# mlvlab/BLiM

Measured on AMD Instinct MI355X. Metric: candidate-pairs/sec (7B, 96+32 tok), higher is better.
Workload: dtype f16; 1 GPU; SYN v2t-VTG re-rank: Qwen2-7B dims (28 layers), seeded synthetic weights, 96 video + 32 text tokens per pair, top-16 text candidates per video query, 55 queries (880 pairs, 32560 packed tokens, 28160 label rows) per step per GPU; prefix_reuse=True, vtg_compensated=none, parallelism=query rows sharded over 1 GPU(s); RCCL all-gather of score rows at the end

## Files before the change

blim_amd/csrc/engine.hip:

```cpp
#include <math.h>
#include <stdarg.h>
#include <stdio.h>
#include <stdlib.h>
#include <string.h>

#include <algorithm>
#include <map>
#include <string>
#include <vector>

#include "engine.hpp"

static thread_local char g_err[1024] = "";
void blim_set_error(const char* fmt, ...) {
    va_list ap;
    va_start(ap, fmt);
    vsnprintf(g_err, sizeof(g_err), fmt, ap);
    va_end(ap);
}
extern "C" const char* blim_last_error(void) { return g_err; }
extern "C" int blim_abi_version(void) { return BLIM_ABI_VERSION; }

static const char* kTimeClassNames[TC_COUNT] = {"gemm_qkv_rope", "attention", "gemm_o_resid", "gemm_gateup_swiglu", "gemm_down_resid",
                                                "rmsnorm", "lm_head_lse", "gemm_other", "misc", "quantize_fp8"};
// ... 1406 lines not shown
        hipEventDestroy(s.a); hipEventDestroy(s.b);
    }
    e->spans.clear();
    return BLIM_OK;
}
extern "C" int blim_debug_read(blim_engine* e, const char* which, void* dst, int64_t bytes, void* stream) {
    ARG_CHECK(e && which && dst && bytes > 0);
    const DevBuf* b = nullptr;
    if (!strcmp(which, "resid")) b = &e->resid;
    else if (!strcmp(which, "xn")) b = &e->xn;
    else if (!strcmp(which, "qkv")) b = &e->qkv;
    else if (!strcmp(which, "attn")) b = &e->attn;
    else if (!strcmp(which, "act")) b = &e->act;
    else if (!strcmp(which, "act8")) b = &e->act8;
    else if (!strcmp(which, "act_mx")) b = &e->act_mx;
    if (!b || !b->p || (size_t)bytes > b->bytes) { blim_set_error("debug_read: no buffer '%s' of %lld bytes", which, (long long)bytes); return BLIM_ERR_ARG; }
    HIP_TRY(hipMemcpyAsync(dst, b->p, (size_t)bytes, hipMemcpyDeviceToDevice, (hipStream_t)stream));
    return BLIM_OK;
}
extern "C" int blim_debug_gemm_stamps(void* device_buf) {
    gemm_set_debug_stamps((unsigned long long*)device_buf);
    return BLIM_OK;
}
extern "C" int blim_set_option(blim_engine* e, const char* key, int32_t value) {
    ARG_CHECK(e && key);
    if (!strcmp(key, "attn_tr_read")) { e->attn_tr = value; return BLIM_OK; }
    if (!strcmp(key, "f8_mask")) { e->f8_mask = value & 31; return BLIM_OK; }
    if (!strcmp(key, "f8_fuse")) { e->f8_fuse = value != 0; return BLIM_OK; }
    if (!strcmp(key, "precise_embeds")) { e->precise_embeds = value != 0; return BLIM_OK; }
    if (!strcmp(key, "prune_last")) { e->prune_last = value != 0; return BLIM_OK; }
    if (!strcmp(key, "masked_query_zero")) {
        if (value && e->f8) { blim_set_error("option 'masked_query_zero' needs a 16-bit engine (the fp8 mode's attention output leaves the kernel quantised)"); return BLIM_ERR_ARG; }
        e->masked_query_zero = value != 0; return BLIM_OK;
    }
    if (!strcmp(key, "precise_lo6")) {
        if (value && e->f8) { blim_set_error("option 'precise_lo6' needs a 16-bit engine (fp16: the default; bf16: opt-in)"); return BLIM_ERR_ARG; }
        if (value && (e->c.hidden_size % 128 || e->c.intermediate_size % 128 || e->c.hidden_size > 20480 || e->c.intermediate_size > 20480)) {
            blim_set_error("option 'precise_lo6': hidden and intermediate sizes must be multiples of 128, at most 20480"); return BLIM_ERR_ARG; }
        if (value && e->aug && e->aug % 128) { blim_set_error("option 'precise_lo6': adapters were loaded with a %d-column K extension; set the option before loading adapters", e->aug); return BLIM_ERR_STATE; }
        e->lo6 = value != 0; return BLIM_OK;
    }
    if (!strcmp(key, "precise_mlp")) { e->precise_mlp = value != 0; return BLIM_OK; }
    if (!strcmp(key, "precise_layers")) {
        if (value && e->f8) { blim_set_error("option 'precise_layers' needs a 16-bit engine (fp16 or bf16)"); return BLIM_ERR_ARG; }
        e->layer_mask_on = value != 0; return BLIM_OK;
    }
// ... 16 lines not shown
```

blim_amd/csrc/gemm.hip:

```cpp
#include "gemm.hpp"
#include "kernels.hpp"
#include <type_traits>

#define BM 256
#define BN 256
#define BK 64
#define NTHREADS 512
#define TILE_BYTES (BM * BK * 2)
#define BUF_BYTES (2 * TILE_BYTES)
#define GROUP_M 8

typedef const __attribute__((address_space(1))) void* gptr_t;
typedef __attribute__((address_space(3))) void* lptr_t;

__device__ __forceinline__ void glds16(const void* g, char* lds_wave_base) {
    __builtin_amdgcn_global_load_lds((gptr_t)g, (lptr_t)lds_wave_base, 16, 0, 0);
}

__device__ __forceinline__ float gelu_erf(float x) {
    const float z = fabsf(x) * 0.70710678118654752f;
    const float t = __builtin_amdgcn_rcpf(fmaf(0.3275911f, z, 1.0f));
    const float poly = t * fmaf(t, fmaf(t, fmaf(t, fmaf(t, 1.061405429f, -1.453152027f), 1.421413741f), -0.284496736f), 0.254829592f);
    const float erf_abs = 1.0f - poly * __expf(-z * z);
    return 0.5f * x * (1.0f + copysignf(erf_abs, x));
}
__device__ __forceinline__ float silu_f(float x) { return x * __builtin_amdgcn_rcpf(1.0f + __expf(-x)); }

template <int EPI, int DT, bool SPLIT = false, bool MXA = false>
__global__ __launch_bounds__(NTHREADS) void gemm_kernel(const GemmParams p) {
    __shared__ __attribute__((aligned(16))) char smem[5 * TILE_BYTES];

    constexpr bool LO6_BF16_FENCE = MXA && DT == DT_BF16;
    const int tid = threadIdx.x;
    const int lane = tid & 63;
    const int wave = __builtin_amdgcn_readfirstlane(tid >> 6);
    const int wm = wave >> 2, wn = wave & 3;
    int stamp_vb = blockIdx.x;
    auto stamp = [&](int k) __attribute__((always_inline)) {
        if (p.debug_stamps && tid == 0) p.debug_stamps[(size_t)stamp_vb * 8 + k] = __builtin_amdgcn_s_memrealtime();
    };
    const int ntm = (p.M + BM - 1) / BM, ntn = (p.N + BN - 1) / BN;
    const int nwg = ntm * ntn;
#pragma unroll 1
    for (int vb = blockIdx.x; vb < (p.tile_map ? ((nwg + 255) & ~255) : nwg); vb += gridDim.x) {
    int pid;
    if (p.tile_map) {
        const int xcd = vb & 7, k = vb >> 3;
        pid = ((k >> 5) * 8 + xcd) * 32 + (k & 31);
        if (pid >= nwg) continue;
    } else {
        const int bid = vb, xcd = bid & 7, q = nwg >> 3, r = nwg & 7;
        pid = (xcd < r ? xcd * (q + 1) : r * (q + 1) + (xcd - r) * q) + (bid >> 3);
    }
    stamp_vb = pid;
    stamp(0);
    if constexpr (out16<DT>::value == DT_F16 || (LO6_BF16_FENCE)) { if (p.f16_saturate) f16_saturate_off(); }
    const int width = p.group_m * ntn;
    const int first_m = (pid / width) * p.group_m;
    const int gsz = min(ntm - first_m, p.group_m);
    const int tm = first_m + (pid % width) % gsz;
    const int tn = (pid % width) / gsz;
    const int row0 = tm * BM, col0 = tn * BN;

    const int sr = lane >> 3;
    const char* baseA = (const char*)p.A;
    const char* baseW = (const char*)p.W;

    constexpr int ES = (DT == DT_F8) ? 1 : 2;
    constexpr bool MX8 = MXA && DT == DT_F8;
    constexpr bool LO6 = MXA && DT != DT_F8;
    constexpr int ODT = out16<DT>::value;
    const int fr = lane & 15, fc = lane >> 4;
    const int fg = (fr >> 1) & 7;
    const int frag_off = (fr >> 3) * 1024 + (fr & 7) * 128 + 16 * ((fc ^ (fg & 3)) + 4 * (fg >> 2));
    const int a_off = (16 * wm) * 1024 + frag_off;
    const int b_off = (8 * wn) * 1024 + frag_off;

    f32x4 acc[8][4];
#pragma unroll
    for (int i = 0; i < 8; ++i)
#pragma unroll
        for (int j = 0; j < 4; ++j) acc[i][j] = (f32x4){0.f, 0.f, 0.f, 0.f};

    const int nk = p.K * ES / (BK * 2);
    const int nk6 = LO6 ? p.K6 / 128 : 0;
    float f8_scale = 0.f;
    if constexpr (DT == DT_F8) f8_scale = tid < 256 ? (p.row_scale ? p.row_scale[min(row0 + tid, p.M - 1)] : 1.0f) : p.col_scale[min(col0 + tid - 256, p.N - 1)];
    stamp(1);
    {
        const int grp = wave >> 2;
        typedef int i32x8 __attribute__((ext_vector_type(8)));
        typedef int i32x4 __attribute__((ext_vector_type(4)));
        bf16x8 fa[2][8], fb[2][4];
        i32x8 fa8[8], fb8[4];
        auto load_frags = [&](int offA_tile, int offB_tile) __attribute__((always_inline)) {
            const char* ba[2] = {smem + (offA_tile + a_off), smem + ((offA_tile + a_off) ^ 64)};
            const char* bb[2] = {smem + (offB_tile + b_off), smem + ((offB_tile + b_off) ^ 64)};
            if constexpr (DT == DT_F8) {
                auto rd = [](const char* q0, const char* q1) __attribute__((always_inline)) {
                    const i32x4 l = *(const i32x4*)q0, h = *(const i32x4*)q1;
                    return (i32x8){l[0], l[1], l[2], l[3], h[0], h[1], h[2], h[3]};
                };
#pragma unroll
                for (int ni = 0; ni < 4; ++ni) fb8[ni] = rd(bb[0] + ni * 2048, bb[1] + ni * 2048);
#pragma unroll
                for (int mi = 0; mi < 8; ++mi) fa8[mi] = rd(ba[0] + mi * 2048, ba[1] + mi * 2048);
            } else {
#pragma unroll
// ... 54 lines not shown
        const int sc = (lane & 7) ^ (4 * (wg & 1) + (sr >> 1));
        uint32_t off8[8];
#pragma unroll
        for (int i = 0; i < 8; ++i) {
            const int b = wg + 4 * i;
            if (grp == 1) off8[i] = (uint32_t)((int64_t)min(row0 + 8 * b + sr, p.M - 1) * p.lda * ES + 16 * sc);
            else off8[i] = (uint32_t)((int64_t)min(col0 + 8 * b + sr, p.N - 1) * (p.w_wrap_k > 0 ? p.w_wrap_k : p.K) * ES + 16 * sc);
        }
        const char* gbase = grp == 1 ? baseA : baseW;
        const int wrap = (grp == 0 && p.w_wrap_k > 0) ? p.w_wrap_k * ES / (BK * 2) : 0x7fffffff;
        auto stage8 = [&](int dst, int kt) __attribute__((always_inline)) {
#ifdef GEMM_ABLATE_DMA
            if (GEMM_ABLATE_DMA == 1 && kt >= 2) return;
            if (GEMM_ABLATE_DMA == 2) kt &= 1;
#endif
            const char* g = gbase + (int64_t)(kt >= wrap ? kt - wrap : kt) * (BK * 2);
#pragma unroll
            for (int i = 0; i < 8; ++i) {
                uint32_t o = off8[i];
                asm volatile("" : "+v"(o));
                glds16(g + o, smem + dst + (wg + 4 * i) * 1024);
            }
        };
        auto frags_and_dma = [&](int offA_tile, int offB_tile, int dst, int kt, bool on) __attribute__((always_inline)) {
            const char* ba[2] = {smem + (offA_tile + a_off), smem + ((offA_tile + a_off) ^ 64)};
            const char* bb[2] = {smem + (offB_tile + b_off), smem + ((offB_tile + b_off) ^ 64)};
#ifdef GEMM_ABLATE_DMA
            if (GEMM_ABLATE_DMA == 1 && kt >= 2) on = false;
            if (GEMM_ABLATE_DMA == 2) kt &= 1;
#endif
#if defined(GEMM_ABLATE_WREAD) && GEMM_ABLATE_WREAD == 2
            if (grp == 0 && kt >= 4) on = false;
#endif
            const char* g = gbase + (int64_t)(kt >= wrap ? kt - wrap : kt) * (BK * 2);
            auto dma1 = [&](int q) __attribute__((always_inline)) {
                __builtin_amdgcn_sched_barrier(0);
                if (on) { uint32_t o = off8[q]; asm volatile("" : "+v"(o)); glds16(g + o, smem + dst + (wg + 4 * q) * 1024); }
                __builtin_amdgcn_sched_barrier(0);
            };
            {
#pragma unroll
                for (int q = 0; q < 8; ++q) {
#pragma unroll
                    for (int j = 3 * q; j < 3 * q + 3; ++j) {
                        const int ks = j / 12, r = j % 12;
#ifdef GEMM_ABLATE_WREAD
                        if (r < 4) { }
#else
                        if (r < 4) fb[ks][r] = *(const bf16x8*)(bb[ks] + r * 2048);
#endif
                        else fa[ks][r - 4] = *(const bf16x8*)(ba[ks] + (r - 4) * 2048);
                    }
                    dma1(q);
                }
#ifdef GEMM_ABLATE_WREAD
#pragma unroll
                for (int ks = 0; ks < 2; ++ks)
#pragma unroll
                    for (int r = 0; r < 4; ++r) fb[ks][r] = fa[ks][r + 4];
#endif
            }
        };
        typedef int i32x2 __attribute__((ext_vector_type(2)));
        const char* g6A = LO6 ? (const char*)p.A6 + (int64_t)tm * nk6 * F6_TILE_BYTES : nullptr;
        const char* g6W = LO6 ? (const char*)p.W6 + (int64_t)tn * nk6 * F6_TILE_BYTES : nullptr;
        uint2 sc6a = make_uint2(0, 0);
        uint32_t sc6w = 0;
        auto dma6 = [&](int q, int dslot, int kd, bool isW, bool on) __attribute__((always_inline)) {
#if defined(GEMM_ABLATE_P2) && GEMM_ABLATE_P2 == 3
            on = on && kd < 3;
#endif
#if defined(GEMM_ABLATE_P2) && GEMM_ABLATE_P2 >= 4
            on = on && !((q == 4 || q == 5) && (isW || GEMM_ABLATE_P2 == 5));
#endif
            if (on) {
                const char* g = (isW ? g6W : g6A) + (int64_t)kd * F6_TILE_BYTES;
                char* d = smem + dslot * F6_TILE_BYTES;
                uint32_t o16 = (uint32_t)lane * 16u;
                asm volatile("" : "+v"(o16));
                if (q < 6) glds16(g + (wg + 4 * q) * 1024 + o16, d + (wg + 4 * q) * 1024);
                else if (lane < 16) glds16(g + 24576 + wg * 256 + o16, d + 24576 + wg * 256);
            }
        };
// ... 35 lines not shown
            stage8(TILE_BYTES, 0);
            if (nk > 1) stage8(3 * TILE_BYTES, 1);
            if (nk > 1) asm volatile("s_waitcnt vmcnt(8)" ::: "memory");
            else asm volatile("s_waitcnt vmcnt(0)" ::: "memory");
            PHASE_BARRIER();
            if constexpr (MX8) mx_cur = mx_nxt;
            if constexpr (DT == DT_F8) {
                int sp = 0;
                for (int k = 0; k < nk; ++k) {
                    mx_request(k + 1);
                    load_frags(sa, adv(sa, 1));
                    if (k >= 1 && k + 1 < nk) stage8(sp, k + 1);
                    PHASE_BARRIER();
                    compute();
                    asm volatile("s_waitcnt vmcnt(0)" ::: "memory");
                    if constexpr (MX8) mx_cur = mx_nxt;
                    PHASE_BARRIER();
                    sp = sa; sa = adv(sa, 2);
                }
                PHASE_BARRIER();
            } else {
            load_frags(0, TILE_BYTES);
            PHASE_BARRIER();
            for (int kt = 0; kt < nk; ++kt) {
                WP_T(0);
                compute();
                WP_T(1);
                asm volatile("s_waitcnt vmcnt(0)" ::: "memory");
                WP_T(2);
                PHASE_BARRIER();
                WP_T(3);
                if constexpr (LO6) { if (kt + 1 == nk) break; }
                if (kt + 1 < nk) frags_and_dma(adv(sa, 2), adv(sa, 3), sa, kt + 2, kt + 2 < nk);
#ifdef GEMM_WAIT_PROF
                asm volatile("s_waitcnt lgkmcnt(0)" ::: "memory");
#endif
                WP_T(4);
                PHASE_BARRIER();
                WP_T(5);
                WP_ACC();
                sa = adv(sa, 2);
            }
            if constexpr (LO6) {
                stage6(0, 0, false); stage6(1, 0, true);
                if (nk6 > 1) { stage6(2, 1, false); stage6(3, 1, true); }
                if (nk6 > 2) { stage6(4, 2, false); stage6(5, 2, true); }
                PHASE_BARRIER();
            }
            }
        } else {
            stage8(0, 0);
            if (nk > 1) stage8(2 * TILE_BYTES, 1);
            if (nk > 1) asm volatile("s_waitcnt vmcnt(8)" ::: "memory");
            else asm volatile("s_waitcnt vmcnt(0)" ::: "memory");
            PHASE_BARRIER();
            if constexpr (MX8) mx_cur = mx_nxt;
            PHASE_BARRIER();
            for (int kt = 0; kt < nk; ++kt) {
                WP_T(0);
                if constexpr (DT == DT_F8) {
                    mx_request(kt + 1);
                    load_frags(sa, adv(sa, 1));
                    if (kt + 2 < nk) stage8(adv(sa, 4), kt + 2);
                } else frags_and_dma(sa, adv(sa, 1), adv(sa, 4), kt + 2, kt + 2 < nk);
#ifdef GEMM_WAIT_PROF
                asm volatile("s_waitcnt lgkmcnt(0)" ::: "memory");
#endif
                WP_T(1);
                if (kt + 2 < nk) asm volatile("s_waitcnt vmcnt(8)" ::: "memory");
                else asm volatile("s_waitcnt vmcnt(0)" ::: "memory");
                WP_T(2);
                PHASE_BARRIER();
                WP_T(3);
                compute();
                if constexpr (MX8) mx_cur = mx_nxt;
                WP_T(4);
                PHASE_BARRIER();
                WP_T(5);
                WP_ACC();
                sa = adv(sa, 2);
            }
        }
        if constexpr (LO6) {
#define P2_VMCNT(n) asm volatile("s_waitcnt vmcnt(" #n ")" ::: "memory")
#define P2_BARRIER() PHASE_BARRIER()
            if (grp == 0) {
                if (nk6 > 2) P2_VMCNT(28);
                else if (nk6 > 1) P2_VMCNT(14);
                else P2_VMCNT(0);
            }
            P2_BARRIER();
            const int qoa = 8 * wm * 1536 + lane * 16, qoa8 = 8 * wm * 1536 + 1024 + lane * 8;
            const int qob = F6_TILE_BYTES + 4 * wn * 1536 + lane * 16, qob8 = F6_TILE_BYTES + 4 * wn * 1536 + 1024 + lane * 8;
            sc6w = rd6_sw(smem + F6_TILE_BYTES); sc6a = rd6_sa(smem);
            fb8[0] = RD6W(smem + qob, smem + qob8, 0); fb8[1] = RD6W(smem + qob, smem + qob8, 1536);
#pragma unroll
            for (int i = 0; i < 4; ++i) fa8[i] = RD6A(smem + qoa, smem + qoa8, i * 1536);
            int s3 = 0;
#ifdef GEMM_WAIT_PROF
            for (int q_ = 0; q_ < 5; ++q_) wp_acc[q_] = 0;
#endif
#if defined(GEMM_ABLATE_P2) && GEMM_ABLATE_P2 == 1
#define L6_MMA(MI, NI)
#else
#define L6_MMA(MI, NI) acc[MI][NI] = __builtin_amdgcn_mfma_scale_f32_16x16x128_f8f6f4(fb8[NI], fa8[MI], acc[MI][NI], 2, 2, NI, (int)sc6w, (MI & 3), (int)((MI) < 4 ? sc6a.x : sc6a.y));
// ... 155 lines not shown
            sm += __shfl_xor(sm, 16); sm += __shfl_xor(sm, 32);
            if (q4 == 0) red[wn * 256 + rl] = make_float2(mx, sm);
        }
        __syncthreads();
        if (tid_e < 256) {
            const int row = row0 + tid_e;
            if (row < p.M) {
                float2 a0 = red[tid_e], a1 = red[256 + tid_e], a2 = red[512 + tid_e], a3 = red[768 + tid_e];
                const float mx = fmaxf(fmaxf(a0.x, a1.x), fmaxf(a2.x, a3.x));
                float sm = 0.f;
                if (mx > -INFINITY) {
                    sm = a0.y * __expf(a0.x - mx) + a1.y * __expf(a1.x - mx) + a2.y * __expf(a2.x - mx) + a3.y * __expf(a3.x - mx);
                }
                p.lse_part[(int64_t)row * ntn + tn] = make_float2(mx, sm);
            }
        }
        stamp(3);
        __syncthreads();
        continue;
    } else {
        int tq = lane >> 4;
        int rsub = lane & 15;
        asm volatile("" : "+v"(tq), "+v"(rsub));
        __syncthreads();
        if constexpr (EPI == EPI_BF16 || EPI == EPI_QKV || EPI == EPI_SWIGLU) {
            constexpr int NC = (EPI == EPI_SWIGLU) ? 128 : 256;
            constexpr int RS = NC * 2 + 16;
            if constexpr (EPI == EPI_SWIGLU && DT == DT_F8) {
                if (p.out_mx != nullptr) {
                    float* red = (float*)smem;
                    uint8_t* st8 = (uint8_t*)smem + 8192;
                    constexpr int RS8 = 144;
#pragma unroll
                    for (int mi = 0; mi < 8; ++mi) {
                        float m = 0.f;
#pragma unroll
                        for (int pr = 0; pr < 2; ++pr)
#pragma unroll
                            for (int j = 0; j < 4; ++j) {
                                const float x = silu_f(acc[mi][2 * pr][j]) * acc[mi][2 * pr + 1][j];
                                acc[mi][2 * pr][j] = x;
                                m = fmaxf(m, fabsf(x));
                            }
                        m = fmaxf(m, __shfl_xor(m, 16)); m = fmaxf(m, __shfl_xor(m, 32));
                        if (tq == 0) red[wn * 256 + 128 * wm + 16 * mi + rsub] = m;
                    }
                    __syncthreads();
// ... 66 lines not shown
            float4 bf16_bias[4];
            if constexpr (EPI == EPI_BF16) {
#pragma unroll
                for (int ni = 0; ni < 4; ++ni) {
                    const int col = wcol0 + 16 * ni + 4 * tq;
                    bf16_bias[ni] = (p.bias && col + 3 < p.N) ? *(const float4*)(p.bias + col) : make_float4(0.f, 0.f, 0.f, 0.f);
                    if (p.bias && col < p.N && col + 3 >= p.N) {
                        bf16_bias[ni].x = p.bias[col];
                        if (col + 1 < p.N) bf16_bias[ni].y = p.bias[col + 1];
                        if (col + 2 < p.N) bf16_bias[ni].z = p.bias[col + 2];
                    }
                }
            }
            if constexpr (EPI == EPI_QKV) {
                if (wcol0 < p.rope_cols) {
                    const int hl = wn >> 1;
                    const int gbase = (wn & 1) * 2;
                    const int d0 = 16 * gbase + 4 * tq;
                    float4 cs[2][2], sn[2][2];
                    const int64_t cstride = p.rope_stride * 16;
                    auto request = [&](int mi, int buf) __attribute__((always_inline)) {
                        const int row = min(row0 + 128 * wm + 16 * (mg0 + mi) + rsub, p.M - 1);
                        const float* base = p.rope_rows + (int64_t)row * 16 + 4 * tq;
                        cs[buf][0] = *(const float4*)(base + (gbase + 0) * cstride); cs[buf][1] = *(const float4*)(base + (gbase + 1) * cstride);
                        sn[buf][0] = *(const float4*)(base + (4 + gbase + 0) * cstride); sn[buf][1] = *(const float4*)(base + (4 + gbase + 1) * cstride);
                    };
                    request(0, 0);
#pragma unroll
                    for (int mi = 0; mi < NMI; ++mi) {
                        if (mi + 1 < NMI) request(mi + 1, (mi + 1) & 1);
                        __builtin_amdgcn_sched_barrier(0);
                        char* lrow = smem + (lrow0 + 16 * mi + rsub) * RS;
#pragma unroll
                        for (int pr = 0; pr < 2; ++pr) {
                            const float4 c = cs[mi & 1][pr], sv = sn[mi & 1][pr];
                            const float c4[4] = {c.x, c.y, c.z, c.w}, s4[4] = {sv.x, sv.y, sv.z, sv.w};
                            const float4 b0 = qkv_bias[2 * pr], b1 = qkv_bias[2 * pr + 1];
                            const float bl[4] = {b0.x, b0.y, b0.z, b0.w}, bh[4] = {b1.x, b1.y, b1.z, b1.w};
                            float lo[4], hi[4];
#pragma unroll
                            for (int j = 0; j < 4; ++j) {
                                const float x1 = acc[mi][2 * pr][j] + bl[j];
                                const float x2 = acc[mi][2 * pr + 1][j] + bh[j];
                                lo[j] = x1 * c4[j] - x2 * s4[j];
                                hi[j] = x2 * c4[j] + x1 * s4[j];
                            }
// ... 163 lines not shown
#pragma unroll
                        for (int j = 0; j < 8; ++j)
                            if (oc + j < n_out) o_[j] = (bf16_t)(w_[j >> 1] >> (16 * (j & 1)));
                    }
                };
                store8(out, v);
                if (SPLIT && !lo_as_tiles) store8(out + p.lo_off, *(const uint4*)(smem + LO_OFF + rl * RS + seg * 16));
                if constexpr (EPI == EPI_BF16 && !SPLIT) {
                    if (p.swiglu_act != nullptr && (seg & 3) < 2) {
                        constexpr int ODT = out16<DT>::value;
                        const uint4 ur = *(const uint4*)(smem + rl * RS + seg * 16 + 32);
                        const uint16_t* gh = (const uint16_t*)&v; const uint16_t* uh = (const uint16_t*)&ur;
                        uint4 o; uint16_t* po = (uint16_t*)&o;
#pragma unroll
                        for (int e = 0; e < 8; ++e) { const float g = from16<ODT>(gh[e]); po[e] = to16<ODT>(silu_f(g) * from16<ODT>(uh[e])); }
                        *(uint4*)(p.swiglu_act + (int64_t)row * p.swiglu_act_ld + oc0 / 2 + 16 * (seg >> 2) + 8 * (seg & 3)) = o;
                    }
                }
            }
            stamp(5);
            }
        } else {
            constexpr int RS = 1024 + 16;
#pragma unroll 1
            for (int h = 0; h < 2; ++h) {
                if (wm == h) {
#pragma unroll
                    for (int mi = 0; mi < 8; ++mi) {
                        char* lrow = smem + (16 * mi + rsub) * RS;
#pragma unroll
                        for (int ni = 0; ni < 4; ++ni) {
                            *(float4*)(lrow + (64 * wn + 16 * ni + 4 * tq) * 4) = make_float4(acc[mi][ni][0], acc[mi][ni][1], acc[mi][ni][2], acc[mi][ni][3]);
                        }
                    }
                }
                __syncthreads();
                const int col = col0 + 4 * lane;
                const bool vec = (col + 3 < p.N) && ((p.ldc & 3) == 0);
                if constexpr (EPI == EPI_RESID) {
                    const float* rsrc = p.resid_in ? p.resid_in : (const float*)p.C;
                    if (vec) {
                        const float4 rb = p.bias ? *(const float4*)(p.bias + col) : make_float4(0.f, 0.f, 0.f, 0.f);
                        float4 o[16];
#pragma unroll
                        for (int i = 0; i < 16; ++i) {
                            const int row = min(row0 + 128 * h + wave + 8 * i, p.M - 1);
                            o[i] = *(const float4*)(rsrc + (int64_t)row * p.ldc + col);
                        }
#pragma unroll
                        for (int i = 0; i < 16; ++i) {
                            const int rl = wave + 8 * i;
                            const int row = row0 + 128 * h + rl;
                            const float4 v = *(const float4*)(smem + rl * RS + lane * 16);
                            if (row < p.M) *(float4*)((float*)p.C + (int64_t)row * p.ldc + col) = make_float4(o[i].x + (v.x + rb.x), o[i].y + (v.y + rb.y), o[i].z + (v.z + rb.z), o[i].w + (v.w + rb.w));
#ifdef GEMM_ABLATE_NORMFOLD
                            if (p.swiglu_act != nullptr && row < p.M) {
                                const float4 nv = make_float4(o[i].x + (v.x + rb.x), o[i].y + (v.y + rb.y), o[i].z + (v.z + rb.z), o[i].w + (v.w + rb.w));
                                float ss = nv.x * nv.x + nv.y * nv.y + nv.z * nv.z + nv.w * nv.w;
#pragma unroll
                                for (int m_ = 1; m_ < 64; m_ <<= 1) ss += __shfl_xor(ss, m_);
                                const float r = rsqrtf(ss * (1.0f / 256.0f) + 1e-6f);
                                const float4 wv = *(const float4*)(p.col_scale + col);
                                const uint16_t h0 = to16<ODT>(nv.x * wv.x * r), h1 = to16<ODT>(nv.y * wv.y * r), h2 = to16<ODT>(nv.z * wv.z * r), h3 = to16<ODT>(nv.w * wv.w * r);
                                *(uint2*)(p.swiglu_act + (int64_t)row * p.swiglu_act_ld + col) = make_uint2((uint32_t)h0 | ((uint32_t)h1 << 16), (uint32_t)h2 | ((uint32_t)h3 << 16));
                                if (lane == 0) ((float*)p.lse_part)[(int64_t)row * ntn + tn] = ss;
                            }
#endif
                        }
                    } else {
#pragma unroll 1
                        for (int i = 0; i < 16; ++i) {
                            const int rl = wave + 8 * i;
                            const int row = row0 + 128 * h + rl;
                            if (row >= p.M || col >= p.N) continue;
                            const float4 v = *(const float4*)(smem + rl * RS + lane * 16);
                            const float x[4] = {v.x, v.y, v.z, v.w};
// ... 1 lines not shown
                            const float* in = rsrc + (int64_t)row * p.ldc + col;
#pragma unroll
                            for (int j = 0; j < 4; ++j)
                                if (col + j < p.N) out[j] = in[j] + x[j] + (p.bias ? p.bias[col + j] : 0.f);
                        }
                    }
                } else {
#pragma unroll 4
                    for (int i = 0; i < 16; ++i) {
                        const int rl = wave + 8 * i;
                        const int row = row0 + 128 * h + rl;
                        if (row >= p.M || col >= p.N) continue;
                        const float4 v = *(const float4*)(smem + rl * RS + lane * 16);
                        float x[4] = {v.x * p.scale, v.y * p.scale, v.z * p.scale, v.w * p.scale};
                        float* out = (float*)p.C + (int64_t)row * p.ldc + col;
                        if (vec) *(float4*)out = make_float4(x[0], x[1], x[2], x[3]);
                        else {
#pragma unroll
                            for (int j = 0; j < 4; ++j)
                                if (col + j < p.N) out[j] = x[j];
                        }
                    }
                }
                __syncthreads();
            }
        }
        if (p.debug_stamps) asm volatile("s_waitcnt vmcnt(0)" ::: "memory");
        stamp(3);
        __syncthreads();
    }
    }
}

#include <stdlib.h>
#include <algorithm>
static int g_gemm_persistent = getenv("BLIM_GEMM_PERSISTENT") ? atoi(getenv("BLIM_GEMM_PERSISTENT")) : 1;
static int g_gemm_tile_map = getenv("BLIM_GEMM_TILE_MAP") ? atoi(getenv("BLIM_GEMM_TILE_MAP")) : -1;
static int g_gemm_group_m = getenv("BLIM_GEMM_GROUP_M") ? atoi(getenv("BLIM_GEMM_GROUP_M")) : GROUP_M;
static int g_f16_saturate = getenv("BLIM_F16_SATURATE") ? atoi(getenv("BLIM_F16_SATURATE")) : 1;
static int g_gemm_skip_epi = getenv("BLIM_GEMM_SKIP_EPI") ? atoi(getenv("BLIM_GEMM_SKIP_EPI")) : 0;
static unsigned long long* g_gemm_stamps = nullptr;
static int g_stamp_epi = getenv("BLIM_GEMM_STAMP_EPI") ? atoi(getenv("BLIM_GEMM_STAMP_EPI")) : -1;
static int g_stamp_k = getenv("BLIM_GEMM_STAMP_K") ? atoi(getenv("BLIM_GEMM_STAMP_K")) : -1;
void gemm_set_debug_stamps(unsigned long long* buf) { g_gemm_stamps = buf; }

template <int EPI>
static int launch_t(const GemmParams& p, hipStream_t stream) {
    const int ntm = (p.M + BM - 1) / BM, ntn = (p.N + BN - 1) / BN;
    static int n_cu = 0;
    if (n_cu == 0) {
        int dev = 0;
        if (hipGetDevice(&dev) != hipSuccess || hipDeviceGetAttribute(&n_cu, hipDeviceAttributeMultiprocessorCount, dev) != hipSuccess || n_cu <= 0) n_cu = 256;
        n_cu = (n_cu / 8) * 8;
        if (n_cu < 8) n_cu = 8;
    }
    const int persistent = g_gemm_persistent ? n_cu : ntm * ntn;
    const dim3 grid(ntm * ntn < persistent ? ntm * ntn : persistent);
    if constexpr (EPI == EPI_QKV || EPI == EPI_SWIGLU || EPI == EPI_RESID || EPI == EPI_LSE) {
        if (p.A6) {
#define LO6_LAUNCH(DTX)                                                                                                                                  \
            if constexpr (EPI == EPI_RESID || EPI == EPI_LSE) hipLaunchKernelGGL((gemm_kernel<EPI, DTX, false, true>), grid, dim3(NTHREADS), 0, stream, p);   \
            else if (p.lo_off != 0) hipLaunchKernelGGL((gemm_kernel<EPI, DTX, true, true>), grid, dim3(NTHREADS), 0, stream, p);                            \
// ... 53 lines not shown
        q.A = (const bf16_t*)((const char*)p.A + r0 * row_bytes);
        if (p.C) q.C = (char*)p.C + r0 * p.ldc * c_es;
        if (p.row_scale) q.row_scale = p.row_scale + r0;
        if (p.rope_rows) q.rope_rows = p.rope_rows + r0 * 16;
        if (p.a_mx) q.a_mx = p.a_mx + r0;
        if (p.out_mx) q.out_mx = p.out_mx + r0;
        if (p.A6) q.A6 = p.A6 + (r0 / BM) * (int64_t)(p.K6 / 128) * F6_TILE_BYTES;
        if (p.out6) q.out6 = p.out6 + (r0 / BM) * (int64_t)(p.N / BN) * F6_TILE_BYTES;
        if (p.labels) q.labels = p.labels + r0;
        if (p.lse_part) q.lse_part = p.lse_part + r0 * ntn;
        if (p.label_logit) q.label_logit = p.label_logit + r0;
        if (p.resid_in) q.resid_in = p.resid_in + r0 * p.ldc;
        if (p.swiglu_gu) q.swiglu_gu = p.swiglu_gu + r0 * p.swiglu_ld;
        if (p.swiglu_act) q.swiglu_act = p.swiglu_act + r0 * p.swiglu_act_ld;
        const int rc = launch_one(epi, q, stream);
        if (rc != BLIM_OK) return rc;
    }
    return BLIM_OK;
}

static int launch_one(GemmEpi epi, const GemmParams& p_in, hipStream_t stream) {
    GemmParams p = p_in;
    p.debug_skip_epilogue = g_gemm_skip_epi;
    static const int dbg_k6 = getenv("BLIM_GEMM_LO6_K6") ? atoi(getenv("BLIM_GEMM_LO6_K6")) : 0;
    if (p.A6 && dbg_k6 > 0 && dbg_k6 < p.K6) p.K6 = dbg_k6;
    if (!g_f16_saturate) p.f16_saturate = 0;
    p.group_m = g_gemm_group_m > 0 ? g_gemm_group_m : GROUP_M;
    const int64_t n_tiles = (int64_t)((p.M + BM - 1) / BM) * ((p.N + BN - 1) / BN);
    p.tile_map = g_gemm_tile_map >= 0 ? g_gemm_tile_map : (((p.N + BN - 1) / BN <= 32 && n_tiles >= 256) ? 1 : 0);
    p.debug_stamps = ((g_stamp_epi < 0 || g_stamp_epi == (int)epi) && (g_stamp_k < 0 || g_stamp_k == p.K)) ? g_gemm_stamps : nullptr;
    ARG_CHECK(p.M > 0 && p.N > 0 && p.K > 0);
    ARG_CHECK(p.A && p.W);
    ARG_CHECK(p.dtype == DT_BF16 || p.dtype == DT_F16 || p.dtype == DT_F8);
    const int es = p.dtype == DT_F8 ? 1 : 2;
    ARG_CHECK((int64_t)p.K * es % 128 == 0);
    ARG_CHECK(p.lda * es % 16 == 0);
    ARG_CHECK(p.dtype != DT_F8 || ((p.row_scale || p.a_mx) && p.col_scale));
    ARG_CHECK((!p.a_mx && !p.out_mx) || (p.dtype == DT_F8 && p.mx_stride >= (int64_t)((p.M + BM - 1) / BM) * 256));
    ARG_CHECK(!p.a_mx || epi == EPI_RESID);
    ARG_CHECK(!p.A6 || ((p.dtype == DT_F16 || p.dtype == DT_BF16) && p.W6 && p.w_wrap_k == 0 && p.K6 > 0 && p.K6 % 128 == 0 && (epi == EPI_RESID || epi == EPI_QKV || epi == EPI_SWIGLU || epi == EPI_LSE)));
    ARG_CHECK(!p.out_mx || (epi == EPI_SWIGLU && p.N % 256 == 0 && p.ldc % 16 == 0));
    ARG_CHECK(!p.out6 || (epi == EPI_SWIGLU && p.A6 && p.lo_off > 0 && p.N % 256 == 0));
    ARG_CHECK(p.w_wrap_k == 0 || (p.K == 2 * p.w_wrap_k && (int64_t)p.w_wrap_k * es % 128 == 0));
    ARG_CHECK(p.lo_off == 0 || epi == EPI_BF16 || epi == EPI_QKV || epi == EPI_SWIGLU);
    ARG_CHECK((int64_t)p.M * p.lda * es < (1ll << 32) && (int64_t)p.N * (p.w_wrap_k > 0 ? p.w_wrap_k : p.K) * es < (1ll << 32));
    switch (epi) {
        case EPI_BF16:
            ARG_CHECK(p.C && p.ldc % 4 == 0);
            ARG_CHECK(!p.swiglu_gu || (p.N % 16 == 0 && p.swiglu_ld % 8 == 0 && p.swiglu_ld >= 2 * (int64_t)p.N));
            ARG_CHECK(!p.swiglu_act || (p.N % 32 == 0 && p.swiglu_act_ld % 8 == 0 && p.swiglu_act_ld >= p.N / 2 && !p.swiglu_gu));
            return launch_t<EPI_BF16>(p, stream);
        case EPI_F32: ARG_CHECK(p.C && p.bias == nullptr); return launch_t<EPI_F32>(p, stream);
        case EPI_RESID: ARG_CHECK(p.C && p.ldc % 4 == 0); return launch_t<EPI_RESID>(p, stream);
        case EPI_QKV:
            ARG_CHECK(p.C && p.bias && p.rope_rows && p.rope_stride >= p.M && p.N % 128 == 0 && p.rope_cols % 128 == 0 && p.ldc % 4 == 0);
            return launch_t<EPI_QKV>(p, stream);
        case EPI_SWIGLU: ARG_CHECK(p.C && p.N % 32 == 0 && p.ldc % 4 == 0); return launch_t<EPI_SWIGLU>(p, stream);
        case EPI_LSE: ARG_CHECK(p.labels && p.lse_part && p.label_logit); return launch_t<EPI_LSE>(p, stream);
    }
    blim_set_error("unknown epilogue %d", (int)epi);
    return BLIM_ERR_ARG;
}
```

blim_amd/csrc/gemm.hpp:

```cpp
#pragma once
#include "common.hpp"

enum GemmEpi : int {
    EPI_BF16 = 0,
    EPI_F32 = 1,
    EPI_RESID = 2,
    EPI_QKV = 3,
    EPI_SWIGLU = 4,
    EPI_LSE = 5,
};

struct GemmParams {
    int dtype;
    const float* row_scale;
    const float* col_scale;
    const bf16_t* A;
    int64_t lda;
    const bf16_t* W;
    int M, N, K;
    void* C;
    int64_t ldc;
    const float* bias;
    const float* resid_in;
    uint16_t* swiglu_gu;
    int64_t swiglu_ld;
    uint16_t* swiglu_act;
    int64_t swiglu_act_ld;
    int act;
    float scale;
    int rope_cols;
    const float* rope_rows;
    int64_t rope_stride;
    const int32_t* labels;
    float2* lse_part;
    float* label_logit;
    int w_wrap_k;
    int64_t lo_off;
    uint8_t* out_mx;
    const uint8_t* a_mx;
    int64_t mx_stride;
    const uint8_t* A6;
    const uint8_t* W6;
    int K6;
    uint8_t* out6;
    int f16_saturate;
    int group_m;
    int tile_map;
    int debug_skip_epilogue;
    unsigned long long* debug_stamps;
};
void gemm_set_debug_stamps(unsigned long long* buf);

int launch_gemm(GemmEpi epi, const GemmParams& p, hipStream_t stream);

static inline int qkv_perm_row(int cprime) { return 16 * (cprime >> 5) + (cprime & 15) + 64 * ((cprime >> 4) & 1); }
```

blim_amd/engine.py:

```python
from __future__ import annotations

import ctypes as C
import os
import re
from typing import Dict, Optional, Sequence

import numpy as np

from .synth import ModelDims, weight_shapes

_HERE = os.path.dirname(os.path.abspath(__file__))
LIB_PATH = os.environ.get("BLIM_LIB_PATH") or os.path.join(_HERE, "libblim_hip.so")
HEADER_PATH = os.path.join(os.path.dirname(_HERE), "include", "blim.h")

DTYPE_F32, DTYPE_BF16 = 0, 1
COMPUTE_DTYPES = {"bf16": 0, "f16": 1, "f8": 2}
DEFAULT_COMPUTE_DTYPE = os.environ.get("BLIM_DTYPE", "f16")


def torch_dtype_of(name: str):
    import torch
    return {"bf16": torch.bfloat16, "f16": torch.float16, "f8": torch.float16}[name]


# ... 58 lines not shown
        "blim_visual_head_f32": ([vp, vp, i64, vp, vp], C.c_int),
        "blim_tvg_scores": ([vp, vp, vp, i32, vp, i32, vp, vp], C.c_int),
        "blim_tvg_logits": ([vp, vp, vp, i32, i32, vp, vp], C.c_int),
        "blim_set_video_vocab": ([vp, vp, i32, vp], C.c_int),
        "blim_tvg_logits_f32": ([vp, vp, i32, vp, vp], C.c_int),
        "blim_score_vtg": ([vp, C.POINTER(Batch), vp, vp, vp, i64, vp, i32, vp, vp], C.c_int),
        "blim_score_tvg": ([vp, C.POINTER(Batch), vp, vp, vp, i32, vp, i32, vp, vp], C.c_int),
        "blim_forward": ([vp, vp, vp, i32, i32, vp, vp, vp], C.c_int),
        "blim_fill_bell_bf16": ([vp, i64, u64, C.c_char_p, f32, f32, vp], C.c_int),
        "blim_fill_bell_f32": ([vp, i64, u64, C.c_char_p, f32, f32, i32, vp], C.c_int),
        "blim_gemm_bf16": ([vp, i64, vp, i32, i32, i32, vp, i64, vp], C.c_int),
        "blim_gemm_f16": ([vp, i64, vp, i32, i32, i32, vp, i64, vp], C.c_int),
        "blim_f6_tiles_bytes": ([i64, i32], C.c_int64),
        "blim_gemm_f16_lo6": ([vp, vp, i32, i32, i32, vp, vp, vp, vp], C.c_int),
        "blim_quant_rows": ([vp, i64, i64, i32, i32, vp, vp, vp], C.c_int),
        "blim_gemm_f8": ([vp, i64, vp, vp, vp, i32, i32, i32, vp, i64, vp], C.c_int),
        "blim_timing_enable": ([vp, i32], C.c_int),
        "blim_timing_num_classes": ([], C.c_int),
        "blim_timing_class_name": ([i32], C.c_char_p),
        "blim_timing_report": ([vp, C.POINTER(C.c_double), C.POINTER(C.c_int64), C.POINTER(C.c_double)], C.c_int),
        "blim_set_option": ([vp, C.c_char_p, i32], C.c_int),
        "blim_debug_read": ([vp, C.c_char_p, vp, i64, vp], C.c_int),
        "blim_debug_gemm_stamps": ([vp], C.c_int),
        "blim_hash_device": ([vp, i64, vp, vp], C.c_int),
        "blim_weights_fingerprint": ([vp, vp, vp], C.c_int),
        "blim_prefix_cache_bytes": ([vp, i32, i32, i32], C.c_int64),
        "blim_prefix_cache_create": ([vp, i32, i32, i32, C.POINTER(vp)], C.c_int),
        "blim_prefix_cache_destroy": ([vp], None),
        "blim_prefix_cache_fill": ([vp, vp, C.POINTER(Batch), vp, vp, vp], C.c_int),
        "blim_prefix_cache_slot_len": ([vp, i32], C.c_int),
        "blim_score_vtg_cached": ([vp, vp, C.POINTER(Batch), vp, vp, i32, vp, vp, vp, i64, vp, i32, vp, vp], C.c_int),
    }
    for name, (args, res) in sig.items():
        fn = getattr(lib, name)
        fn.argtypes = args
        fn.restype = res
    _lib = lib
    return lib


def _check(rc: int, what: str):
    if rc != 0:
        raise BlimError(f"{what} failed (code {rc}): {load_library().blim_last_error().decode()}")


def _ptr(t) -> int:
# ... 439 lines not shown
def gemm_f16_lo6(a_hilo, w):
    import torch
    lib = load_library()
    M, K2 = a_hilo.shape
    N, K = w.shape
    assert K2 == 2 * K and a_hilo.dtype == torch.float16 and w.dtype == torch.float16 and a_hilo.is_contiguous() and w.is_contiguous()
    a6 = torch.empty(lib.blim_f6_tiles_bytes(M, K), dtype=torch.uint8, device=w.device)
    w6 = torch.empty(lib.blim_f6_tiles_bytes(N, K), dtype=torch.uint8, device=w.device)
    out = torch.empty((M, N), dtype=torch.float32, device=w.device)
    _check(lib.blim_gemm_f16_lo6(_ptr(a_hilo), _ptr(w), M, N, K, _ptr(a6), _ptr(w6), _ptr(out), _stream()), "blim_gemm_f16_lo6")
    return out, a6.view(-1, K // 128, 25600), w6.view(-1, K // 128, 25600)


def gemm_bf16(a, w):
    import torch
    lib = load_library()
    M, K = a.shape
    N = w.shape[0]
    assert a.dtype == w.dtype and a.dtype in (torch.bfloat16, torch.float16)
    out = torch.empty((M, N), dtype=a.dtype, device=a.device)
    fn = lib.blim_gemm_bf16 if a.dtype == torch.bfloat16 else lib.blim_gemm_f16
    _check(fn(_ptr(a), K, _ptr(w), M, N, K, _ptr(out), N, _stream()), "blim_gemm")
    return out
```

include/blim.h:

```cpp
#ifndef BLIM_H_
#define BLIM_H_
#include <stdint.h>
#ifdef __cplusplus
extern "C" {
#endif

#define BLIM_ABI_VERSION 9
#define BLIM_ERR_ARG (-1)
#define BLIM_ERR_HIP (-2)
#define BLIM_ERR_STATE (-3)
#define BLIM_ERR_NOMEM (-4)

#define BLIM_DTYPE_F32 0
#define BLIM_DTYPE_BF16 1

#define BLIM_COMPUTE_BF16 0
#define BLIM_COMPUTE_F16 1
#define BLIM_COMPUTE_F8 2

typedef struct blim_engine blim_engine;

typedef struct blim_config {
    int32_t vocab_size, hidden_size, intermediate_size, num_layers, num_heads, num_kv_heads;
    int32_t mm_hidden_size;
// ... 75 lines not shown
                          float* score, void* stream);

int blim_forward(blim_engine* e, const void* embeds, const uint8_t* mask, int32_t B, int32_t L, float* logits, float* hidden, void* stream);

int blim_fill_bell_bf16(void* out, int64_t n, uint64_t seed, const char* name, float std, float mean, void* stream);
int blim_fill_bell_f32(float* out, int64_t n, uint64_t seed, const char* name, float std, float mean, int32_t round_bf16, void* stream);
int blim_gemm_f16(const void* A, int64_t lda, const void* W, int32_t M, int32_t N, int32_t K, void* C, int64_t ldc, void* stream);
int blim_gemm_bf16(const void* A, int64_t lda, const void* W, int32_t M, int32_t N, int32_t K, void* C, int64_t ldc, void* stream);
int64_t blim_f6_tiles_bytes(int64_t n_rows, int32_t K);
int blim_gemm_f16_lo6(const void* A_hilo, const void* W, int32_t M, int32_t N, int32_t K, void* a6, void* w6, float* C, void* stream);
int blim_quant_rows(const void* in16, int64_t ld, int64_t n_rows, int32_t K, int32_t dtype16, void* out8, float* scale, void* stream);
int blim_gemm_f8(const void* A8, int64_t lda, const float* a_scale, const void* W8, const float* w_scale, int32_t M, int32_t N, int32_t K,
                 void* C, int64_t ldc, void* stream);

int blim_timing_enable(blim_engine* e, int32_t on);
int blim_timing_num_classes(void);
const char* blim_timing_class_name(int32_t cls);
int blim_timing_report(blim_engine* e, double* ms, int64_t* calls, double* flops);

int blim_debug_read(blim_engine* e, const char* which, void* dst, int64_t bytes, void* stream);

int blim_debug_gemm_stamps(void* device_buf);

int blim_set_option(blim_engine* e, const char* key, int32_t value);

typedef struct blim_vision blim_vision;
typedef struct blim_vision_config {
    int32_t image_size;
    int32_t patch_size;
    int32_t num_frames;
    int32_t hidden_size;
    int32_t num_heads;
    int32_t mlp_hidden;
    int32_t depth;
    int32_t tome_tokens;
    int32_t compute_dtype;
} blim_vision_config;
int blim_vision_create(const blim_vision_config* cfg, blim_vision** out);
void blim_vision_destroy(blim_vision* v);
int blim_vision_load_weight(blim_vision* v, const char* name, const void* data, int32_t dtype, int32_t on_device);
int blim_vision_init_synthetic_weights(blim_vision* v, uint64_t seed);
int blim_vision_set_pos_embed(blim_vision* v, const float* table_host);
int blim_vision_ready(const blim_vision* v);
int blim_vision_encode(blim_vision* v, const void* frames, int32_t n_clips, float* out_feat, float* out_tome, void* stream);
int blim_vit_attention(const void* qkv, int32_t n_clips, int32_t L, int32_t heads, int32_t dtype16, void* out, void* stream);
int blim_tome_merge(blim_vision* v, const float* x, int32_t b, int32_t p, int32_t c, int32_t heads, int32_t target, float* out, void* stream);
// ... 42 lines not shown
```

Measured before the change: 2595 pairs/s.

## Prefetch residual rows into LDS during final K iterations of residual GEMM

For the residual-add epilogue (o_proj and down_proj), the GEMM now starts DMA loads of the first residual row block into the freed LDS ring during the last two K iterations. The epilogue then streams the remaining residual blocks through LDS in a four-stage pipeline, adding accumulators in place and writing out coalesced rows. The aim is to hide residual read latency behind the tail of the main loop and drop the separate stage-then-read pass. It also replaces __syncthreads with lighter lgkmcnt+s_barrier syncs, and adds an env toggle and a debug entry point for comparing the two paths. The cost is more intricate LDS slot bookkeeping and a fast path limited to full tiles without bias.

After: 2601 pairs/s (median of 6 runs). About the same (+0.2%).

```diff
diff --git a/blim_amd/csrc/engine.hip b/blim_amd/csrc/engine.hip
--- a/blim_amd/csrc/engine.hip
+++ b/blim_amd/csrc/engine.hip
@@ -1452,6 +1452,15 @@
     gemm_set_debug_stamps((unsigned long long*)device_buf);
     return BLIM_OK;
 }
+extern "C" int blim_debug_gemm_epi(int32_t epi, int32_t prefetch, int32_t dtype16, const void* A, int64_t lda, const void* W, int32_t M, int32_t N, int32_t K, float* C, int64_t ldc,
+                                   const float* resid_in, const float* bias, void* stream) {
+    ARG_CHECK(A && W && C && (dtype16 == DT_BF16 || dtype16 == DT_F16) && (prefetch == 0 || prefetch == 1));
+    if (epi != (int32_t)EPI_RESID) { blim_set_error("debug_gemm_epi: only the residual epilogue (%d) has two paths", (int)EPI_RESID); return BLIM_ERR_ARG; }
+    GemmParams p = gp(dtype16, A, lda, W, M, N, K, C, ldc);
+    p.resid_in = resid_in; p.bias = bias;
+    p.epi_prefetch = prefetch ? 2 : 1;
+    return launch_gemm(EPI_RESID, p, (hipStream_t)stream);
+}
 extern "C" int blim_set_option(blim_engine* e, const char* key, int32_t value) {
     ARG_CHECK(e && key);
     if (!strcmp(key, "attn_tr_read")) { e->attn_tr = value; return BLIM_OK; }
diff --git a/blim_amd/csrc/gemm.hip b/blim_amd/csrc/gemm.hip
--- a/blim_amd/csrc/gemm.hip
+++ b/blim_amd/csrc/gemm.hip
@@ -32,7 +32,7 @@
 
     constexpr bool LO6_BF16_FENCE = MXA && DT == DT_BF16;
     const int tid = threadIdx.x;
-    const int lane = tid & 63;
+    constexpr bool PF_OK = EPI == EPI_RESID && !SPLIT && !MXA && DT != DT_F8;
     const int wave = __builtin_amdgcn_readfirstlane(tid >> 6);
     const int wm = wave >> 2, wn = wave & 3;
     int stamp_vb = blockIdx.x;
@@ -43,6 +43,9 @@
     const int nwg = ntm * ntn;
 #pragma unroll 1
     for (int vb = blockIdx.x; vb < (p.tile_map ? ((nwg + 255) & ~255) : nwg); vb += gridDim.x) {
+    int lane_t = tid & 63;
+    if constexpr (PF_OK) asm volatile("" : "+v"(lane_t));
+    const int lane = lane_t;
     int pid;
     if (p.tile_map) {
         const int xcd = vb & 7, k = vb >> 3;
@@ -84,6 +87,9 @@
 
     const int nk = p.K * ES / (BK * 2);
     const int nk6 = LO6 ? p.K6 / 128 : 0;
+    bool epf = false;
+    if constexpr (PF_OK) epf = p.epi_prefetch && nk >= 3 && row0 + BM <= p.M && col0 + BN <= p.N && (p.ldc & 3) == 0 && p.bias == nullptr;
+    int epi_img = 0;
     float f8_scale = 0.f;
     if constexpr (DT == DT_F8) f8_scale = tid < 256 ? (p.row_scale ? p.row_scale[min(row0 + tid, p.M - 1)] : 1.0f) : p.col_scale[min(col0 + tid - 256, p.N - 1)];
     stamp(1);
@@ -184,6 +190,15 @@
                 glds16(g + o, smem + dst + (wg + 4 * i) * 1024);
             }
         };
+        constexpr int ERS = 1024 + 16, ECELLS = RING / ERS;
+        auto epi_c0 = [](int img) { const int slot = img >> 15; return 32 * slot - (slot >= 3 ? 1 : 0); };
+        auto epi_cell = [](int c0, int j) { const int c = c0 + j; return (c >= ECELLS ? c - ECELLS : c) * ERS; };
+        auto resid_req = [&](int c0, int ps, int il) __attribute__((always_inline)) {
+            const float* g = (p.resid_in ? p.resid_in : (const float*)p.C) + (int64_t)(row0 + 128 * (il >> 5) + 32 * ps + (il & 31)) * p.ldc + col0;
+            uint32_t o = (uint32_t)lane * 16u;
+            asm volatile("" : "+v"(o));
+            glds16((const char*)g + o, smem + epi_cell(c0, 64 * (ps & 1) + il));
+        };
         auto frags_and_dma = [&](int offA_tile, int offB_tile, int dst, int kt, bool on) __attribute__((always_inline)) {
             const char* ba[2] = {smem + (offA_tile + a_off), smem + ((offA_tile + a_off) ^ 64)};
             const char* bb[2] = {smem + (offB_tile + b_off), smem + ((offB_tile + b_off) ^ 64)};
@@ -194,7 +209,9 @@
 #if defined(GEMM_ABLATE_WREAD) && GEMM_ABLATE_WREAD == 2
             if (grp == 0 && kt >= 4) on = false;
 #endif
-            const char* g = gbase + (int64_t)(kt >= wrap ? kt - wrap : kt) * (BK * 2);
+            int kw = kt >= wrap ? kt - wrap : kt;
+            if constexpr (PF_OK) asm volatile("" : "+s"(kw));
+            const char* g = gbase + (int64_t)kw * (BK * 2);
             auto dma1 = [&](int q) __attribute__((always_inline)) {
                 __builtin_amdgcn_sched_barrier(0);
                 if (on) { uint32_t o = off8[q]; asm volatile("" : "+v"(o)); glds16(g + o, smem + dst + (wg + 4 * q) * 1024); }
@@ -221,6 +238,23 @@
 #pragma unroll
                     for (int r = 0; r < 4; ++r) fb[ks][r] = fa[ks][r + 4];
 #endif
+            }
+        };
+        auto frags_and_resid = [&](int offA_tile, int offB_tile, int rimg) __attribute__((always_inline)) {
+            const char* ba[2] = {smem + (offA_tile + a_off), smem + ((offA_tile + a_off) ^ 64)};
+            const char* bb[2] = {smem + (offB_tile + b_off), smem + ((offB_tile + b_off) ^ 64)};
+            const int c0 = epi_c0(rimg);
+#pragma unroll
+            for (int q = 0; q < 8; ++q) {
+#pragma unroll
+                for (int j = 3 * q; j < 3 * q + 3; ++j) {
+                    const int ks = j / 12, r = j % 12;
+                    if (r < 4) fb[ks][r] = *(const bf16x8*)(bb[ks] + r * 2048);
+                    else fa[ks][r - 4] = *(const bf16x8*)(ba[ks] + (r - 4) * 2048);
+                }
+                __builtin_amdgcn_sched_barrier(0);
+                resid_req(c0, 0, 32 * grp + 4 * q + wg);
+                __builtin_amdgcn_sched_barrier(0);
             }
         };
         typedef int i32x2 __attribute__((ext_vector_type(2)));
@@ -302,7 +336,8 @@
             } else {
             load_frags(0, TILE_BYTES);
             PHASE_BARRIER();
-            for (int kt = 0; kt < nk; ++kt) {
+            const int nkl0 = (PF_OK && epf) ? nk - 2 : nk;
+            for (int kt = 0; kt < nkl0; ++kt) {
                 WP_T(0);
                 compute();
                 WP_T(1);
@@ -321,6 +356,20 @@
                 WP_ACC();
                 sa = adv(sa, 2);
             }
+            if constexpr (PF_OK) {
+                if (epf) {
+                    compute();
+                    asm volatile("s_waitcnt vmcnt(0)" ::: "memory");
+                    PHASE_BARRIER();
+                    frags_and_resid(adv(sa, 2), adv(sa, 3), adv(sa, 4));
+                    PHASE_BARRIER();
+                    sa = adv(sa, 2);
+                    compute();
+                    PHASE_BARRIER();
+                    PHASE_BARRIER();
+                    sa = adv(sa, 2);
+                }
+            }
             if constexpr (LO6) {
                 stage6(0, 0, false); stage6(1, 0, true);
                 if (nk6 > 1) { stage6(2, 1, false); stage6(3, 1, true); }
@@ -336,7 +385,8 @@
             PHASE_BARRIER();
             if constexpr (MX8) mx_cur = mx_nxt;
             PHASE_BARRIER();
-            for (int kt = 0; kt < nk; ++kt) {
+            const int nkl1 = (PF_OK && epf) ? nk - 1 : nk;
+            for (int kt = 0; kt < nkl1; ++kt) {
                 WP_T(0);
                 if constexpr (DT == DT_F8) {
                     mx_request(kt + 1);
@@ -360,7 +410,17 @@
                 WP_ACC();
                 sa = adv(sa, 2);
             }
+            if constexpr (PF_OK) {
+                if (epf) {
+                    frags_and_resid(sa, adv(sa, 1), adv(sa, 2));
+                    PHASE_BARRIER();
+                    compute();
+                    PHASE_BARRIER();
+                    sa = adv(sa, 2);
+                }
+            }
         }
+        if constexpr (PF_OK) epi_img = sa;
         if constexpr (LO6) {
 #define P2_VMCNT(n) asm volatile("s_waitcnt vmcnt(" #n ")" ::: "memory")
 #define P2_BARRIER() PHASE_BARRIER()
@@ -562,7 +622,9 @@
         int tq = lane >> 4;
         int rsub = lane & 15;
         asm volatile("" : "+v"(tq), "+v"(rsub));
-        __syncthreads();
+#define TILE_SYNC()                                                                                                                \
+        do { if constexpr (PF_OK) { asm volatile("s_waitcnt lgkmcnt(0)" ::: "memory"); __builtin_amdgcn_s_barrier(); asm volatile("" ::: "memory"); } else __syncthreads(); } while (0)
+        if (!(PF_OK && epf)) TILE_SYNC();
         if constexpr (EPI == EPI_BF16 || EPI == EPI_QKV || EPI == EPI_SWIGLU) {
             constexpr int NC = (EPI == EPI_SWIGLU) ? 128 : 256;
             constexpr int RS = NC * 2 + 16;
@@ -675,6 +737,10 @@
                     auto request = [&](int mi, int buf) __attribute__((always_inline)) {
                         const int row = min(row0 + 128 * wm + 16 * (mg0 + mi) + rsub, p.M - 1);
                         const float* base = p.rope_rows + (int64_t)row * 16 + 4 * tq;
+#if defined(GEMM_ABLATE_EPI) && GEMM_ABLATE_EPI == 2
+                        cs[buf][0] = cs[buf][1] = make_float4(0.8f, 0.8f, 0.8f, 0.8f); sn[buf][0] = sn[buf][1] = make_float4(0.6f, 0.6f, 0.6f, 0.6f);
+                        return;
+#endif
                         cs[buf][0] = *(const float4*)(base + (gbase + 0) * cstride); cs[buf][1] = *(const float4*)(base + (gbase + 1) * cstride);
                         sn[buf][0] = *(const float4*)(base + (4 + gbase + 0) * cstride); sn[buf][1] = *(const float4*)(base + (4 + gbase + 1) * cstride);
                     };
@@ -884,6 +950,64 @@
             }
         } else {
             constexpr int RS = 1024 + 16;
+            if constexpr (PF_OK) {
+                if (epf) {
+#define EPI_BARRIER()                                          \
+                    asm volatile("s_waitcnt lgkmcnt(0)" ::: "memory"); \
+                    __builtin_amdgcn_s_barrier();                      \
+                    asm volatile("" ::: "memory")
+                    constexpr int ERS = RS, ECELLS = 5 * TILE_BYTES / ERS;
+                    int c0 = 32 * (epi_img >> 15) - ((epi_img >> 15) >= 3 ? 1 : 0);
+                    auto cell = [&](int j) __attribute__((always_inline)) { const int c = c0 + j; return (c >= ECELLS ? c - ECELLS : c) * ERS; };
+                    const float* rsrc = p.resid_in ? p.resid_in : (const float*)p.C;
+#pragma unroll
+                    for (int ps = 0; ps < 4; ++ps) {
+                        if (ps + 1 < 4) {
+#pragma unroll
+                            for (int i = 0; i < 8; ++i) {
+                                const int il = wave + 8 * i;
+                                const float* g = rsrc + (int64_t)(row0 + 128 * (il >> 5) + 32 * (ps + 1) + (il & 31)) * p.ldc + col0;
+                                uint32_t o = (uint32_t)lane * 16u;
+                                asm volatile("" : "+v"(o));
+                                glds16((const char*)g + o, smem + cell(64 * ((ps + 1) & 1) + il));
+                            }
+                        }
+                        if (ps == 0 || ps == 3) asm volatile("s_waitcnt vmcnt(8)" ::: "memory");
+                        else asm volatile("s_waitcnt vmcnt(16)" ::: "memory");
+                        EPI_BARRIER();
+#pragma unroll
+                        for (int m2 = 0; m2 < 2; ++m2) {
+                            char* lrow = smem + cell(64 * (ps & 1) + 32 * wm + 16 * m2 + rsub) + (64 * wn + 4 * tq) * 4;
+                            f32x4 r[4];
+#pragma unroll
+                            for (int ni = 0; ni < 4; ++ni) r[ni] = *(const f32x4*)(lrow + 64 * ni);
+                            __builtin_amdgcn_sched_barrier(0);
+#pragma unroll
+                            for (int ni = 0; ni < 4; ++ni) *(f32x4*)(lrow + 64 * ni) = r[ni] + acc[2 * ps + m2][ni];
+                            __builtin_amdgcn_sched_barrier(0);
+                        }
+                        EPI_BARRIER();
+#pragma unroll
+                        for (int i0 = 0; i0 < 8; i0 += 4) {
+                            f32x4 v[4];
+#pragma unroll
+                            for (int i = 0; i < 4; ++i) v[i] = *(const f32x4*)(smem + cell(64 * (ps & 1) + wave + 8 * (i0 + i)) + lane * 16);
+                            __builtin_amdgcn_sched_barrier(0);
+#pragma unroll
+                            for (int i = 0; i < 4; ++i) {
+                                const int il = wave + 8 * (i0 + i);
+                                *(f32x4*)((float*)p.C + (int64_t)(row0 + 128 * (il >> 5) + 32 * ps + (il & 31)) * p.ldc + col0 + 4 * lane) = v[i];
+                            }
+                            __builtin_amdgcn_sched_barrier(0);
+                        }
+                        EPI_BARRIER();
+                    }
+#undef EPI_BARRIER
+                    if (p.debug_stamps) asm volatile("s_waitcnt vmcnt(0)" ::: "memory");
+                    stamp(3);
+                    continue;
+                }
+            }
 #pragma unroll 1
             for (int h = 0; h < 2; ++h) {
                 if (wm == h) {
@@ -892,11 +1016,11 @@
                         char* lrow = smem + (16 * mi + rsub) * RS;
 #pragma unroll
                         for (int ni = 0; ni < 4; ++ni) {
-                            *(float4*)(lrow + (64 * wn + 16 * ni + 4 * tq) * 4) = make_float4(acc[mi][ni][0], acc[mi][ni][1], acc[mi][ni][2], acc[mi][ni][3]);
-                        }
-                    }
-                }
-                __syncthreads();
+                            *(f32x4*)(lrow + (64 * wn + 16 * ni + 4 * tq) * 4) = acc[mi][ni];
+                        }
+                    }
+                }
+                TILE_SYNC();
                 const int col = col0 + 4 * lane;
                 const bool vec = (col + 3 < p.N) && ((p.ldc & 3) == 0);
                 if constexpr (EPI == EPI_RESID) {
@@ -907,13 +1031,18 @@
 #pragma unroll
                         for (int i = 0; i < 16; ++i) {
                             const int row = min(row0 + 128 * h + wave + 8 * i, p.M - 1);
+#if defined(GEMM_ABLATE_EPI) && GEMM_ABLATE_EPI == 1
+                            o[i] = make_float4(0.f, 0.f, 0.f, 0.f);
+#else
                             o[i] = *(const float4*)(rsrc + (int64_t)row * p.ldc + col);
+#endif
                         }
 #pragma unroll
                         for (int i = 0; i < 16; ++i) {
                             const int rl = wave + 8 * i;
                             const int row = row0 + 128 * h + rl;
-                            const float4 v = *(const float4*)(smem + rl * RS + lane * 16);
+                            const f32x4 vv = *(const f32x4*)(smem + rl * RS + lane * 16);
+                            const float4 v = make_float4(vv[0], vv[1], vv[2], vv[3]);
                             if (row < p.M) *(float4*)((float*)p.C + (int64_t)row * p.ldc + col) = make_float4(o[i].x + (v.x + rb.x), o[i].y + (v.y + rb.y), o[i].z + (v.z + rb.z), o[i].w + (v.w + rb.w));
 #ifdef GEMM_ABLATE_NORMFOLD
                             if (p.swiglu_act != nullptr && row < p.M) {
@@ -961,12 +1090,13 @@
                         }
                     }
                 }
-                __syncthreads();
+                TILE_SYNC();
             }
         }
         if (p.debug_stamps) asm volatile("s_waitcnt vmcnt(0)" ::: "memory");
         stamp(3);
-        __syncthreads();
+        TILE_SYNC();
+#undef TILE_SYNC
     }
     }
 }
@@ -977,6 +1107,7 @@
 static int g_gemm_tile_map = getenv("BLIM_GEMM_TILE_MAP") ? atoi(getenv("BLIM_GEMM_TILE_MAP")) : -1;
 static int g_gemm_group_m = getenv("BLIM_GEMM_GROUP_M") ? atoi(getenv("BLIM_GEMM_GROUP_M")) : GROUP_M;
 static int g_f16_saturate = getenv("BLIM_F16_SATURATE") ? atoi(getenv("BLIM_F16_SATURATE")) : 1;
+static int g_gemm_epi_prefetch = getenv("BLIM_GEMM_EPI_PREFETCH") ? atoi(getenv("BLIM_GEMM_EPI_PREFETCH")) : 1;
 static int g_gemm_skip_epi = getenv("BLIM_GEMM_SKIP_EPI") ? atoi(getenv("BLIM_GEMM_SKIP_EPI")) : 0;
 static unsigned long long* g_gemm_stamps = nullptr;
 static int g_stamp_epi = getenv("BLIM_GEMM_STAMP_EPI") ? atoi(getenv("BLIM_GEMM_STAMP_EPI")) : -1;
@@ -1076,6 +1207,10 @@
 static int launch_one(GemmEpi epi, const GemmParams& p_in, hipStream_t stream) {
     GemmParams p = p_in;
     p.debug_skip_epilogue = g_gemm_skip_epi;
+    p.epi_prefetch = p_in.epi_prefetch ? p_in.epi_prefetch - 1 : (g_gemm_epi_prefetch != 0);
+#ifdef GEMM_ABLATE_EPI
+    p.epi_prefetch = 0;
+#endif
     static const int dbg_k6 = getenv("BLIM_GEMM_LO6_K6") ? atoi(getenv("BLIM_GEMM_LO6_K6")) : 0;
     if (p.A6 && dbg_k6 > 0 && dbg_k6 < p.K6) p.K6 = dbg_k6;
     if (!g_f16_saturate) p.f16_saturate = 0;
@@ -1105,7 +1240,7 @@
             ARG_CHECK(!p.swiglu_act || (p.N % 32 == 0 && p.swiglu_act_ld % 8 == 0 && p.swiglu_act_ld >= p.N / 2 && !p.swiglu_gu));
             return launch_t<EPI_BF16>(p, stream);
         case EPI_F32: ARG_CHECK(p.C && p.bias == nullptr); return launch_t<EPI_F32>(p, stream);
-        case EPI_RESID: ARG_CHECK(p.C && p.ldc % 4 == 0); return launch_t<EPI_RESID>(p, stream);
+        case EPI_RESID: ARG_CHECK(p.C && p.ldc >= p.N); return launch_t<EPI_RESID>(p, stream);
         case EPI_QKV:
             ARG_CHECK(p.C && p.bias && p.rope_rows && p.rope_stride >= p.M && p.N % 128 == 0 && p.rope_cols % 128 == 0 && p.ldc % 4 == 0);
             return launch_t<EPI_QKV>(p, stream);
diff --git a/blim_amd/csrc/gemm.hpp b/blim_amd/csrc/gemm.hpp
--- a/blim_amd/csrc/gemm.hpp
+++ b/blim_amd/csrc/gemm.hpp
@@ -46,6 +46,7 @@
     int f16_saturate;
     int group_m;
     int tile_map;
+    int epi_prefetch;
     int debug_skip_epilogue;
     unsigned long long* debug_stamps;
 };
diff --git a/blim_amd/engine.py b/blim_amd/engine.py
--- a/blim_amd/engine.py
+++ b/blim_amd/engine.py
@@ -104,6 +104,7 @@
         "blim_set_option": ([vp, C.c_char_p, i32], C.c_int),
         "blim_debug_read": ([vp, C.c_char_p, vp, i64, vp], C.c_int),
         "blim_debug_gemm_stamps": ([vp], C.c_int),
+        "blim_debug_gemm_epi": ([i32, i32, i32, vp, i64, vp, i32, i32, i32, vp, i64, vp, vp, vp], C.c_int),
         "blim_hash_device": ([vp, i64, vp, vp], C.c_int),
         "blim_weights_fingerprint": ([vp, vp, vp], C.c_int),
         "blim_prefix_cache_bytes": ([vp, i32, i32, i32], C.c_int64),
@@ -589,3 +590,16 @@
     fn = lib.blim_gemm_bf16 if a.dtype == torch.bfloat16 else lib.blim_gemm_f16
     _check(fn(_ptr(a), K, _ptr(w), M, N, K, _ptr(out), N, _stream()), "blim_gemm")
     return out
+
+
+def gemm_resid_debug(a, w, resid, prefetch: bool, out=None, bias=None, ldc=None):
+    import torch
+    lib = load_library()
+    M, K = a.shape
+    N = w.shape[0]
+    ldc = N if ldc is None else ldc
+    assert a.dtype == w.dtype and a.dtype in (torch.bfloat16, torch.float16) and resid.dtype == torch.float32 and resid.numel() >= (M - 1) * ldc + N
+    dst = resid if out is None else out
+    _check(lib.blim_debug_gemm_epi(2, 1 if prefetch else 0, 0 if a.dtype == torch.bfloat16 else 1, _ptr(a), K, _ptr(w), M, N, K, _ptr(dst), ldc,
+                                   None if out is None else _ptr(resid), _ptr(bias), _stream()), "blim_debug_gemm_epi")
+    return dst
diff --git a/include/blim.h b/include/blim.h
--- a/include/blim.h
+++ b/include/blim.h
@@ -121,6 +121,9 @@
 
 int blim_debug_gemm_stamps(void* device_buf);
 
+int blim_debug_gemm_epi(int32_t epi, int32_t prefetch, int32_t dtype16, const void* A, int64_t lda, const void* W, int32_t M, int32_t N, int32_t K, float* C, int64_t ldc,
+                        const float* resid_in, const float* bias, void* stream);
+
 int blim_set_option(blim_engine* e, const char* key, int32_t value);
 
 typedef struct blim_vision blim_vision;
```
